# tusen-ai/simpledet

Measured on AMD Instinct MI355X. Metric: images/sec at 800x1333 FPN 512-RoI RoIAlign fwd+bwd, higher is better.
Workload: dtype f32; 1 GPU; fused FPN RoIAlign_v2 fwd+bwd, P2-P5 256ch 800x1333, N=2 img/GPU, 512 RoIs/img, 7x7x4 samples (BASELINE configs[1]); images_per_gpu=2, rois_per_image=512, argmax_state=packed u8 (decoded in backward)

## Files before the change

simpledet_amd/csrc/roi_align_common.h:

```cpp
#pragma once
#include "common.h"
#include "../../include/simpledet_ops.h"
#include <float.h>
#include <math.h>
#include <type_traits>
#include <hip/hip_fp16.h>

namespace sd {

struct RoiLevels {
  const float* data[SD_MAX_FPN_LEVELS];
  int H[SD_MAX_FPN_LEVELS], W[SD_MAX_FPN_LEVELS], stride[SD_MAX_FPN_LEVELS];
  float scale[SD_MAX_FPN_LEVELS];
  int nlvl;
  float canon_scale, canon_level, k_min, k_max;
};

__device__ __forceinline__ int fpn_level(float x1, float y1, float x2, float y2,
                                         const RoiLevels& L) {
  float area = (x2 - x1 + 1.f) * (y2 - y1 + 1.f);
  float s = sqrtf(area);
  float t = floorf(L.canon_level + log2f(s / L.canon_scale + 1e-6f));
  t = t < L.k_min ? L.k_min : (t > L.k_max ? L.k_max : t);
  if (!(t == t)) return -1;
// ... 86 lines not shown
  float* coords;
  int nslice;
  int fbslice;
  int ablate;
  long long* dbg;
  int half_io;
};

__device__ __forceinline__ int axis_samples(int p, int pooled, float start_c, float end_c,
                                            float scale, int size, int mul, float* val, float* frac,
                                            int* off) {
  float roi_start = start_c * scale;
  float roi_end = end_c * scale;
  float roi_len = roi_end - roi_start;
  float bin = roi_len / (float)pooled;
  float lo = (float)p * bin;
  float hi = (float)(p + 1) * bin;
  lo = fminr(fmaxr(lo + roi_start, 0.f), (float)(size - 1));
  hi = fminr(fmaxr(hi + roi_start, 0.f), (float)(size - 1));
  int cnt = -1;
  off[0] = off[1] = off[2] = off[3] = -1;
  if (!(hi <= lo)) {
    cnt = 0;
    float stride = (hi - lo) / 3.0f;
    double lim = (double)(hi - stride) + 0.01;
    float step = fmaxr(stride, 0.01f);
    for (float v = lo + stride; (double)v <= lim; v += step) {
      if (cnt < 2) {
        int low = iminr(imaxr((int)floorf(v), 0), size - 1);
        int high = iminr(imaxr((int)ceilf(v), 0), size - 1);
        val[cnt] = v;
        frac[cnt] = (low == high) ? 0.5f : (v - (float)low);
        off[2 * cnt] = low * mul;
        off[2 * cnt + 1] = high * mul;
      }
      ++cnt;
      if (cnt >= 3) break;
    }
  }
  return cnt;
}

constexpr int kCoordWords = 9;

__device__ __forceinline__ float sample_coord(int p, int pooled, float start_c, float end_c,
                                              float scale, int size, int k) {
  const float roi_start = start_c * scale;
  const float roi_end = end_c * scale;
  const float roi_len = roi_end - roi_start;
  const float bin = roi_len / (float)pooled;
  float lo = (float)p * bin;
  float hi = (float)(p + 1) * bin;
  lo = fminr(fmaxr(lo + roi_start, 0.f), (float)(size - 1));
  hi = fminr(fmaxr(hi + roi_start, 0.f), (float)(size - 1));
  const float stride = (hi - lo) / 3.0f;
  const float step = fmaxr(stride, 0.01f);
  float v = lo + stride;
  for (int i = 0; i < k; ++i) v += step;
  return v;
}

__device__ __forceinline__ void store_tap(float* dst, float v, int size) {
  int packed = -1;
  float frac = 0.f;
  if (v != -1.f) {
    const int lo = iminr(imaxr((int)floorf(v), 0), size - 1);
    const int hi = iminr(imaxr((int)ceilf(v), 0), size - 1);
    frac = (lo == hi) ? 0.5f : (v - (float)lo) / (float)(hi - lo);
    packed = lo | (hi << 16);
  }
  reinterpret_cast<int*>(dst)[0] = packed;
  dst[1] = frac;
}

constexpr int kBandThreads = 1024, kBandWaves = kBandThreads / kWave;
constexpr int kBandBufFloats = 16896;
constexpr int kBandHalo = 8;
constexpr int kBandMaxBands = 16;
constexpr int kBandNP = 4;
constexpr int kBandMaxUnits = 512;
constexpr int kBandFillCost = 140, kBandPlaneCost = 60, kBandSetupCost = 1500;
constexpr int kBandSub = 4;
constexpr int kBandFallbackWGs = 0;

typedef float v2f __attribute__((ext_vector_type(2)));

struct BandPlan {
  int owned[SD_MAX_FPN_LEVELS];
  int rows[SD_MAX_FPN_LEVELS];
  int nbands[SD_MAX_FPN_LEVELS];
  int g[SD_MAX_FPN_LEVELS];
  int unit_base[SD_MAX_FPN_LEVELS];
  int halo[SD_MAX_FPN_LEVELS];
  int nwg;
  int nunits;
  int grab;
  int gbias;
  int tail;
  int tail_planes;
  int pool;
  uint4* rowent;
  uint4* colent;
  float2* rowval;
  float2* colval;
  unsigned* items;
  int2* seg;
  unsigned char* fbflag;
  int* chan_ctr;
  int nlist, nent;
};

struct BandArgs {
  FwdArgs f;
  BandPlan p;
};

struct BwdArgs {
  RoiLevels L;
  const float* dy;
  const float* ax;
  const float* ay;
  const float* rois;
  float* dx;
  int B, C, R, PP, H, W;
  float scale;
  int filter_lvl;
  int band_rows, nbands;
  int req;
  int ablate;
};

struct BwdFusedArgs {
  RoiLevels L;
  const float* dy;
  const float* ax;
  const float* ay;
  const unsigned char* amax8;
  const float* coords;
  const float* rois;
  float* dx[SD_MAX_FPN_LEVELS];
  int band_rows[SD_MAX_FPN_LEVELS], nbands[SD_MAX_FPN_LEVELS];
  int block_end[SD_MAX_FPN_LEVELS];
  int order[SD_MAX_FPN_LEVELS];
  int nlaunch;
  int B, C, R, PP;
  int filter;
  int req;
  int ablate;
  int* ws_list;
  float* ws_taps;
  int unit_base[SD_MAX_FPN_LEVELS];
  int lists_units;
  int half_io;
  int float_adds;
  int pix_bound_words;
};
constexpr int kPixBoundMaxWords = 10240;

constexpr int kListSplit = 4;
constexpr int kMergedListSplit = 2;

int fill_levels(RoiLevels& L, const float* const* feats, const int* Hs, const int* Ws, const int* strides,
                int nlvl, float canon_scale, float canon_level);
int check_dims(int B, int C, int R, int ph, int pw);
int launch_fwd(FwdArgs& a, hipStream_t st, void* workspace = nullptr, size_t workspace_bytes = 0,
               const BwdFusedArgs* bplan = nullptr, bool* bplan_done = nullptr);
int launch_bwd_fused(BwdFusedArgs& a, int nlvl, hipStream_t st, void* workspace = nullptr,
                     size_t workspace_bytes = 0, int prepass = 0);
int launch_bwd(BwdArgs& a, hipStream_t st);
int launch_fwd_prep(const BandArgs& A, int pool, int nblocks, const BwdFusedArgs* bplan, hipStream_t st);
int launch_bwd_lists(const BwdFusedArgs& a, int units, hipStream_t st);

}
```

simpledet_amd/csrc/roi_align_fwd.hip:

```cpp
#include "roi_align_common.h"

namespace sd {

__global__ __launch_bounds__(256) void roi_align_fwd_naive(FwdArgs a) {
  const int PP = a.PH * a.PW;
  const long count = (long)a.B * a.R * a.C * PP;
  for (long index = (long)blockIdx.x * blockDim.x + threadIdx.x; index < count;
       index += (long)gridDim.x * blockDim.x) {
    int pw = (int)(index % a.PW);
    int ph = (int)((index / a.PW) % a.PH);
    int c = (int)((index / PP) % a.C);
    int n = (int)(index / PP / a.C);
    const float* r = a.rois + (long)n * 4;
    float x1 = r[0], y1 = r[1], x2 = r[2], y2 = r[3];
    int lvl = 0;
    if (a.L.nlvl > 1) lvl = fpn_level(x1, y1, x2, y2, a.L);
    FwdOut o{0.f, -1.f, -1.f, 255};
    if (lvl >= 0) {
      int H = a.L.H[lvl], W = a.L.W[lvl];
      const float* plane = a.L.data[lvl] + ((long)(n / a.R) * a.C + c) * H * W;
      o = roi_align_fwd_elem(plane, H, W, x1, y1, x2, y2, a.L.scale[lvl], ph, pw, a.PH, a.PW);
    }
    if (a.L.nlvl > 1) o.val = o.val + 0.0f;
    a.out[index] = o.val;
// ... 349 lines not shown
                      bk = (kl >> 1) * 3 + (kl & 1);
                    } else {
                      bx = cx[b][kl & 1];
                      by = cy[b][kl >> 1];
                    }
                  }
                }
                if (a.L.nlvl > 1) maxval = maxval + 0.0f;
                const int g = bin;
                po[g + d * NWAVE * PPG] = maxval;
                if (PK) {
                  if (!(SD_ABLATE(a, 4))) pk[g + d * NWAVE * PPSG] = (unsigned char)(bk < 0 ? 255 : bk);
                } else {
                  px[g + d * NWAVE * PPG] = bx;
                  py[g + d * NWAVE * PPG] = by;
                }
              }
            }
            wave_lds_sync();
          }
        }
        pl += D * pstep;
        po += D * NWAVE * PPG;
        if (PK) {
          pk += D * NWAVE * PPSG;
        } else {
          px += D * NWAVE * PPG;
          py += D * NWAVE * PPG;
        }
      }
    };
    if (any_dup) channel_loop(std::true_type{});
    else channel_loop(std::false_type{});
  }
}

template <int PH, int PW, int NROI, bool PK>
__global__ __launch_bounds__(512) void roi_align_fwd_tiled(FwdArgs a) {
  __shared__ FwdSmem<PH, PW, NROI> s;
  fwd_tiled_body<PH, PW, NROI, PK>(a, s, blockIdx.x);
}

__device__ __forceinline__ int band_fill(const float* gsrc, int len, float* buf, int wave, int lane) {
  const int shift = (int)(((uintptr_t)gsrc >> 2) & 3);
  const float* a0 = gsrc - shift;
  const int n4 = (shift + len + 3) >> 2;
  const int first_full = shift ? 1 : 0;
  const int last_full = ((shift + len) >> 2);
  const float4* s4 = reinterpret_cast<const float4*>(a0);
  float4* d4 = reinterpret_cast<float4*>(buf);
  for (int w4 = wave * kWave; w4 < last_full; w4 += kBandWaves * kWave) {
    const int i = w4 + lane;
    if (i >= first_full && i < last_full) __builtin_amdgcn_global_load_lds(s4 + i, d4 + w4, 16, 0, 0);
  }
  if (wave == 0) {
    if (shift && lane < 4 && lane >= shift && lane < shift + len)
      __builtin_amdgcn_global_load_lds(a0 + lane, buf, 4, 0, 0);
    if (last_full < n4 && last_full >= first_full && (last_full > 0 || !shift)) {
      const int j = last_full * 4 + lane;
      if (lane < 4 && j < shift + len) __builtin_amdgcn_global_load_lds(a0 + j, buf + last_full * 4, 4, 0, 0);
    }
  }
  return shift;
}

template <int POOL, bool PK, bool HALF = false>
__global__ __launch_bounds__(kBandThreads) void roi_align_fwd_band(BandArgs A) {
  using TIn = typename std::conditional<HALF, __half, float>::type;
  constexpr int AL = HALF ? 8 : 4;
  const FwdArgs& a = A.f;
  const BandPlan& P = A.p;
  constexpr int QL = POOL, IPP = kWave / QL;
  constexpr int NP = (PK && !HALF) ? kBandNP : kBandNP - 1, CAP = NP * kBandWaves * IPP;
  constexpr int PPG = POOL * POOL, PPSG = amax_stride(PPG);
  extern __shared__ __attribute__((aligned(16))) float band_smem[];
  const int tid = threadIdx.x, lane = tid & (kWave - 1);
  const int wave = __builtin_amdgcn_readfirstlane(tid / kWave);

#ifdef SD_PROFILING
  const long long t_entry = __builtin_readcyclecounter();
#endif
  __shared__ int v_unit[kBandMaxUnits], v_first[kBandMaxUnits], v_items[kBandMaxUnits];
  __shared__ int v_cost[kBandMaxUnits], v_start[kBandMaxUnits + 1];
  __shared__ int2 s_grab[2];
  __shared__ int s_pick;
  const int wg = (int)blockIdx.x - kBandFallbackWGs, nwg = (int)gridDim.x - kBandFallbackWGs;
  const int rsub = (a.R + kBandSub - 1) / kBandSub;
  auto level_of = [&](int u) {
    int l = 0;
    for (int k = 0; k < a.L.nlvl; ++k)
      if (a.L.stride[k] >= 0 && u >= P.unit_base[k]) l = k;
    return l;
  };
  __shared__ int s_nvu;
  auto wave_incl_scan = [&](int v) {
#pragma unroll
    for (int o = 1; o < kWave; o <<= 1) {
      const int t = __shfl_up(v, o);
      if (lane >= o) v += t;
    }
    return v;
  };
  static_assert(kBandMaxUnits % kWave == 0 && kBandMaxUnits / kWave <= kBandWaves, "unit table: one wave per 64 units");
  constexpr int NB = kBandMaxUnits / kWave;
  __shared__ int s_tot[NB], s_ctot[NB];
  {
    const int u = wave * kWave + lane;
    int cnt = 0, rounds = 0, lv = 0, incl = 0;
    if (wave < NB) {
      if (u < P.nunits) {
        lv = level_of(u);
#pragma unroll
        for (int j = 0; j < kBandSub; ++j) cnt += P.seg[u * kBandSub + j].y;
        rounds = (cnt + CAP - 1) / CAP;
      }
      incl = wave_incl_scan(rounds);
      if (lane == kWave - 1) s_tot[wave] = incl;
    }
    __syncthreads();
    int total = 0;
#pragma unroll
    for (int b = 0; b < NB; ++b) total += s_tot[b];
    const int n = total < kBandMaxUnits ? total : kBandMaxUnits;
    if (wave < NB) {
      int vb = incl - rounds;
#pragma unroll
      for (int b = 0; b < NB; ++b) vb += b < wave ? s_tot[b] : 0;
      for (int r = 0; r < rounds && vb + r < kBandMaxUnits; ++r) {
        const int it = cnt - r * CAP < CAP ? cnt - r * CAP : CAP;
        v_unit[vb + r] = u;
        v_first[vb + r] = r * CAP;
        v_items[vb + r] = it;
        const int cst = kBandFillCost / P.g[lv] + kBandPlaneCost + it;
        v_cost[vb + r] = P.g[lv] > 1 ? cst + cst * P.gbias / 100 : cst;
      }
    }
    __syncthreads();
    const int v = wave * kWave + lane;
    int mine = 0, cincl = 0;
    if (wave < NB) {
      mine = v < n ? kBandSetupCost + v_cost[v] * a.C : 0;
      cincl = wave_incl_scan(mine);
      if (lane == kWave - 1) s_ctot[wave] = cincl;
    }
    __syncthreads();
    if (wave < NB) {
      int run = cincl - mine;
#pragma unroll
      for (int b = 0; b < NB; ++b) run += b < wave ? s_ctot[b] : 0;
      if (v < n) v_start[v] = run;
      if (v == n - 1 || (n == 0 && v == 0)) v_start[n] = n == 0 ? 0 : run + mine;
    }
    if (tid == 0) s_nvu = n;
  }
  __syncthreads();
  const int nvu = s_nvu;
  int vu = 0;
  {
    const long pos = (long)v_start[nvu] * (2 * wg + 1) / (2 * nwg);
    int below = 0;
    for (int k = lane; k < nvu; k += kWave) below += v_start[k] <= pos ? 1 : 0;
    below = wave_sum_i32(below);
    vu = below > 0 ? below - 1 : 0;
  }
  float* buf0 = band_smem;
  float* buf1 = band_smem + kBandBufFloats;
#ifdef SD_PROFILING
  const long long t_begin = __builtin_readcyclecounter();
  long long t_setup = 0, t_wait = 0, t_comp = 0, t_mark = t_begin;
  int dbg_count = 0, dbg_units = 0, dbg_fills = 0;
#endif
  auto grab = [&](int v, int G) {
    int k = 0;
    if (tid == 0) k = atomicAdd(&P.chan_ctr[v], G);
    return k;
  };

  for (int visit = 0; nvu > 0; ++visit) {
  if (visit) {
    if (wave == 0) {
      int best = -1, bestval = 0;
      for (int v0 = 0; v0 < nvu; v0 += kWave) {
        const int v = v0 + lane;
        int left = 0;
        if (v < nvu) {
          const int done = __hip_atomic_load(&P.chan_ctr[v], __ATOMIC_RELAXED, __HIP_MEMORY_SCOPE_AGENT);
          if (done < a.C && (done == 0 || a.C - done >= 3 * P.g[level_of(v_unit[v])])) {
            left = (a.C - done) * v_cost[v];
            left = left < 1 ? 1 : left;
          }
        }
        int m = left;
#pragma unroll
        for (int o = 32; o >= 1; o >>= 1) {
          const int t = __shfl_xor(m, o);
          m = t > m ? t : m;
        }
        if (m > bestval) {
          bestval = m;
          best = v0 + __builtin_ctzll(__ballot(left == m));
        }
      }
      if (lane == 0) s_pick = best;
    }
    __syncthreads();
    vu = s_pick;
    if (vu < 0) break;
  }
  const int unit = v_unit[vu];
  const int lvl = level_of(unit);
  const int G = P.g[lvl], nb = P.nbands[lvl];
  const int GR = ((P.grab + G - 1) / G) * G;
  int glast = 0;
  auto next_size = [&]() { return glast >= a.C - a.C * P.tail / 100 ? (P.tail_planes < G ? P.tail_planes : G) : GR; };
  {
    const int k = grab(vu, GR);
    if (tid == 0) s_grab[0] = make_int2(k, GR);
    glast = k;
    __syncthreads();
  }
  int kcur = s_grab[0].x;
  if (kcur >= a.C) continue;
  int ck = kcur + G, cend = kcur + GR < a.C ? kcur + GR : a.C;
  int gcur = cend - kcur < G ? cend - kcur : G, gnext = 0;
  int slot = 1;
  const int ul = unit - P.unit_base[lvl];
  const int img = ul / nb, band = ul % nb;
  const int H = a.L.H[lvl], W = a.L.W[lvl], HW = H * W;
  const int r0 = band * P.owned[lvl];
  const int nrows = H - r0 < P.rows[lvl] ? H - r0 : P.rows[lvl];
  const int blen = nrows * W;
  const int bstride = HALF ? ((blen + 14) >> 3) * 8 : (blen + 4 + 3) & ~3;
  const unsigned* items = P.items + ((long)img * SD_MAX_FPN_LEVELS + lvl) * kBandSub * rsub * POOL;
  int sgs[kBandSub], sgc[kBandSub], count = 0;
#pragma unroll
  for (int j = 0; j < kBandSub; ++j) {
    const int2 sg = P.seg[unit * kBandSub + j];
    sgs[j] = j * rsub * POOL + sg.x - count;
    sgc[j] = count + sg.y;
    count += sg.y;
  }
  const int round0 = v_first[vu], nitems = v_items[vu];
#ifdef SD_PROFILING
  dbg_count += nitems;
  ++dbg_units;
  dbg_fills = 0;
  t_mark = __builtin_readcyclecounter();
  if (a.dbg && lane == 0 && wave == 0 && dbg_units <= 3) {
    long long* d = a.dbg + ((long)gridDim.x * kBandWaves + (long)blockIdx.x * 4 + (dbg_units - 1)) * 8;
    d[0] = lvl; d[2] = nitems; d[3] = t_mark; d[4] = 1;
  }
#endif
  const TIn* gbase = reinterpret_cast<const TIn*>(a.L.data[lvl]) + (long)img * a.C * HW + (long)r0 * W;
  {
    constexpr int NST = HALF ? 3 : 1;
    uint4 st[NST];
    const int n8u = (blen + 7 + 7) >> 3;
    auto fill = [&](const TIn* src, float* dst, int gcount) {
      if constexpr (!HALF) {
        int sh0 = 0;
        for (int g = 0; g < gcount; ++g) {
          const int sh = band_fill(src + (long)g * HW, blen, dst + g * bstride, wave, lane);
          if (g == 0) sh0 = sh;
        }
        return sh0;
      } else {
        const int sh0 = (int)(((uintptr_t)src >> 1) & 7);
#pragma unroll
        for (int k = 0; k < NST; ++k) {
          const int f = tid + k * kBandThreads, g = f / n8u, i = f - g * n8u;
          st[k] = make_uint4(0, 0, 0, 0);
          if (g < gcount) {
            const __half* sp = src + (long)g * HW;
            const int sh = (int)(((uintptr_t)sp >> 1) & 7);
            const int e0 = 8 * i - sh;
            if (e0 >= 0 && e0 + 8 <= blen) {
              st[k] = *reinterpret_cast<const uint4*>(sp + e0);
            } else if (e0 + 8 > 0 && e0 < blen) {
              unsigned short h[8];
#pragma unroll
              for (int j = 0; j < 8; ++j)
                h[j] = (e0 + j >= 0 && e0 + j < blen) ? reinterpret_cast<const unsigned short*>(sp)[e0 + j] : 0;
              st[k] = make_uint4(h[0] | (unsigned)h[1] << 16, h[2] | (unsigned)h[3] << 16,
                                 h[4] | (unsigned)h[5] << 16, h[6] | (unsigned)h[7] << 16);
            }
          }
        }
        return sh0;
      }
    };
    auto fill_commit = [&](float* dst, int gcount) {
      if constexpr (HALF) {
#pragma unroll
        for (int k = 0; k < NST; ++k) {
          const int f = tid + k * kBandThreads, g = f / n8u, i = f - g * n8u;
          if (g < gcount) {
            const __half2* hp = reinterpret_cast<const __half2*>(&st[k]);
            const float2 p0 = __half22float2(hp[0]), p1 = __half22float2(hp[1]);
            const float2 p2 = __half22float2(hp[2]), p3 = __half22float2(hp[3]);
            float4* d = reinterpret_cast<float4*>(dst + g * bstride + 8 * i);
            d[0] = make_float4(p0.x, p0.y, p1.x, p1.y);
            d[1] = make_float4(p2.x, p2.y, p3.x, p3.y);
          }
        }
      }
    };
    int A0[NP], A1[NP], A2[NP], A3[NP], A4[NP], A5[NP], A6[NP], A7[NP];
    float al0[NP], al1[NP], be0[NP], be1[NP], cx0[NP], cx1[NP], cy0[NP], cy1[NP];
    int ooff[NP];
    unsigned aoff[NP];
    int flags[NP];
    bool anyd[NP];
    unsigned words[NP];
    uint4 res[NP], ces[NP];
#pragma unroll
    for (int i = 0; i < NP; ++i) {
      const int it = (wave + kBandWaves * i) * IPP + lane / QL;
      const bool valid = lane < IPP * QL && it < nitems;
      words[i] = 0;
      if (valid) {
// ... 414 lines not shown
  L.nlvl = nlvl;
  L.canon_scale = canon_scale;
  L.canon_level = canon_level;
  L.k_min = (float)log2((double)smin);
  L.k_max = (float)log2((double)smax);
  return SD_OK;
}

int launch_fwd(FwdArgs& a, hipStream_t st, void* workspace, size_t workspace_bytes, const BwdFusedArgs* bplan,
               bool* bplan_done) {
  if (bplan_done) *bplan_done = false;
  const long count = (long)a.B * a.R * a.C * a.PH * a.PW;
  if (count == 0) return SD_OK;
  const int variant = tuning("roi_align_fwd", 1);
  a.ablate = SD_PROF_TUNING("roi_align_fwd_ablate", 0);
  a.dbg = reinterpret_cast<long long*>(((uintptr_t)(unsigned)SD_PROF_TUNING("roi_align_dbg_hi", 0) << 32) |
                                       (uintptr_t)(unsigned)SD_PROF_TUNING("roi_align_dbg_lo", 0));
  const int nroi = a.B * a.R;
  a.nslice = 1;
  for (int d = 1; d <= a.C && d <= 8; ++d)
    if (a.C % d == 0) a.nslice = d;
  const int wantfb = a.L.nlvl > 1 ? 32 : 8;
  a.fbslice = 1;
  for (int d = 1; d <= a.C && d <= wantfb; ++d)
    if (a.C % d == 0) a.fbslice = d;
  bool wide = true;
  for (int l = 0; l < a.L.nlvl; ++l)
    if (a.L.stride[l] >= 0 && a.L.W[l] < 2) wide = false;
  if (variant == 1 && wide && ((a.PH == 7 && a.PW == 7) || (a.PH == 14 && a.PW == 14)) &&
      a.R <= 65535 && workspace && tuning("roi_align_fwd_band", 1)) {
    BandArgs A{};
    BandPlan& P = A.p;
    const int POOL = a.PH;
    bool ok = true;
    int units = 0;
    constexpr int gmax = 8;
    int nvalid_lv = 0;
    for (int l = 0; l < a.L.nlvl; ++l) nvalid_lv += a.L.stride[l] >= 0;
    for (int l = 0; l < a.L.nlvl; ++l) {
      if (a.L.stride[l] < 0) continue;
      const int H = a.L.H[l], W = a.L.W[l];
      const long HW = (long)H * W;
      if (W > 4095 || HW >= (1 << 20)) { ok = false; break; }
      int halo = kBandHalo;
      if (H <= 128) {
        halo = (H + POOL - 1) / POOL + 2;
        halo = halo < kBandHalo ? kBandHalo : (halo > 12 ? 12 : halo);
      }
      const int rb = (kBandBufFloats - 16) / W;
      if (rb < halo + 4) { ok = false; break; }
      int nbn = H <= rb ? 1 : (H + (rb - halo) - 1) / (rb - halo);
      const int cap = kBandNP * kBandWaves * (kWave / POOL);
      const long est = (long)a.R * POOL / (nvalid_lv > 0 ? nvalid_lv : 1);
      const int by_items = (int)((est * 5 + 4L * cap - 1) / (4L * cap));
      if (by_items > nbn && a.amax8) nbn = by_items;
      if (nbn > H) nbn = H;
      if (nbn > kBandMaxBands) nbn = kBandMaxBands;
      int owned = (H + nbn - 1) / nbn;
      if (nbn > 1)
        for (int o = owned; o < owned + 4 && o + halo <= rb; ++o)
          if (((long)o * W) % 4 == 0) { owned = o; break; }
      if (owned + halo > rb) owned = rb - halo;
      nbn = (H + owned - 1) / owned;
      if (nbn > kBandMaxBands) { ok = false; break; }
      P.nbands[l] = nbn;
      P.halo[l] = halo;
      P.owned[l] = nbn == 1 ? H : owned;
      P.rows[l] = nbn == 1 ? H : (owned + halo < H ? owned + halo : H);
      const long bstride = a.half_io ? (((long)P.rows[l] * W + 14) >> 3) * 8 : (((long)P.rows[l] * W + 4 + 3) & ~3L);
      int g = 1;
      for (int c = 2; c <= 8 && c <= gmax; c *= 2)
        if (a.C % c == 0 && c * bstride <= kBandBufFloats) g = c;
      if (bstride > kBandBufFloats) { ok = false; break; }
      P.g[l] = g;
      P.unit_base[l] = units;
      units += a.B * P.nbands[l];
    }
    auto al16 = [](size_t x) { return (x + 15) & ~(size_t)15; };
    const size_t ent = al16((size_t)nroi * POOL * sizeof(uint4));
    const size_t valb = a.amax8 ? 0 : al16((size_t)nroi * POOL * sizeof(float2));
    const size_t itemb = al16((size_t)a.B * SD_MAX_FPN_LEVELS * kBandSub * ((a.R + kBandSub - 1) / kBandSub) *
                              POOL * sizeof(unsigned));
    const size_t segb = al16((size_t)units * kBandSub * sizeof(int2));
    const size_t need = 16 + 2 * ent + 2 * valb + itemb + segb + al16(nroi) + kBandMaxUnits * sizeof(int);
    int wg = 0;
    P.nunits = units;
    P.grab = 4;
    P.gbias = 0;
    P.tail = 0;
    P.tail_planes = 8;
    {
      const int np = (a.amax8 && !a.half_io) ? kBandNP : kBandNP - 1;
      const long cap_launch = (long)np * kBandWaves * (kWave / POOL);
      if (units + (long)nroi * POOL / cap_launch > kBandMaxUnits) ok = false;
    }
    wg = kNumCU;
    if (ok && need <= workspace_bytes) {
      char* w = reinterpret_cast<char*>(((uintptr_t)workspace + 15) & ~(uintptr_t)15);
      P.rowent = reinterpret_cast<uint4*>(w); w += ent;
      P.colent = reinterpret_cast<uint4*>(w); w += ent;
      if (valb) {
        P.rowval = reinterpret_cast<float2*>(w); w += valb;
        P.colval = reinterpret_cast<float2*>(w); w += valb;
      }
      P.items = reinterpret_cast<unsigned*>(w); w += itemb;
      P.seg = reinterpret_cast<int2*>(w); w += segb;
      P.fbflag = reinterpret_cast<unsigned char*>(w); w += al16(nroi);
      P.chan_ctr = reinterpret_cast<int*>(w);
      P.nwg = wg;
      P.pool = POOL;
      A.f = a;
      const int nlist = a.B * a.L.nlvl * kBandSub, nent = cdiv((long)nroi * 2 * POOL, kBandThreads);
      const int ncoord = a.amax8 ? cdiv((long)nroi * 6 * POOL, kBandThreads) : 0;
      P.nlist = nlist; P.nent = nent;
      const int smem = 2 * kBandBufFloats * (int)sizeof(float);
      const bool merged = bplan && bplan->lists_units > 0 && bplan->PP == POOL * POOL;
      if (bplan_done) *bplan_done = merged;
      if (int e = launch_fwd_prep(A, POOL, nlist + nent + ncoord, merged ? bplan : nullptr, st)) return e;
      {
        const long HW0 = (long)a.L.H[0] * a.L.W[0];
        const size_t lds = (size_t)(HW0 + 1) * 16 + 8 * 4 * 49 * sizeof(float);
        if (!a.amax8 && !a.half_io && POOL == 7 && a.L.nlvl == 1 && a.L.stride[0] >= 0 && P.nbands[0] == 1 &&
            a.C % 4 == 0 && lds <= 78 * 1024 && a.B <= 65535 &&
            (((uintptr_t)a.L.data[0] | (uintptr_t)a.out | (uintptr_t)a.ax | (uintptr_t)a.ay) & 15) == 0 &&
            tuning("roi_align_fwd_quad", 1) == 1) {
          SD_HIP_CHECK(hipFuncSetAttribute((const void*)roi_align_fwd_quad, hipFuncAttributeMaxDynamicSharedMemorySize, (int)lds));
          hipLaunchKernelGGL(roi_align_fwd_quad, dim3(a.C / 4, a.B), dim3(512), lds, st, A);
          note_dispatch("sd::roi_fwd_prep_kernel<7> + sd::roi_align_fwd_quad");
          SD_LAUNCH_CHECK();
          return SD_OK;
        }
      }
#define SD_FWD_BAND(POOLV, PK)                                                                    \
  do {                                                                                            \
    auto k = roi_align_fwd_band<POOLV, PK>;                                                       \
    SD_HIP_CHECK(hipFuncSetAttribute((const void*)k, hipFuncAttributeMaxDynamicSharedMemorySize,  \
                                     smem));                                                      \
    hipLaunchKernelGGL(k, dim3(wg + kBandFallbackWGs), dim3(kBandThreads), smem, st, A);          \
  } while (0)
      if (a.half_io) {
#define SD_FWD_BAND_H(POOLV)                                                                      \
  do {                                                                                            \
    auto k = roi_align_fwd_band<POOLV, true, true>;                                               \
    SD_HIP_CHECK(hipFuncSetAttribute((const void*)k, hipFuncAttributeMaxDynamicSharedMemorySize,  \
                                     smem));                                                      \
    hipLaunchKernelGGL(k, dim3(wg + kBandFallbackWGs), dim3(kBandThreads), smem, st, A);          \
  } while (0)
        if (POOL == 7) SD_FWD_BAND_H(7); else SD_FWD_BAND_H(14);
#undef SD_FWD_BAND_H
      } else if (POOL == 7) {
        if (a.amax8) SD_FWD_BAND(7, true); else SD_FWD_BAND(7, false);
      } else {
        if (a.amax8) SD_FWD_BAND(14, true); else SD_FWD_BAND(14, false);
      }
#undef SD_FWD_BAND
      note_dispatch("sd::%s<%d> + sd::roi_align_fwd_band<%d,%s,%s>", merged ? "roi_prep_merged_kernel" : "roi_fwd_prep_kernel",
                    POOL, POOL, a.amax8 ? "true" : "false", a.half_io ? "true" : "false");
      SD_LAUNCH_CHECK();
      return SD_OK;
    }
  }
  if (a.half_io)
    return fail(SD_ERR_UNSUPPORTED, "fp16 RoIAlign runs on the band-resident kernel only: it needs the workspace, "
                "7x7 or 14x14 pooling, W in [2, 4095] and roi_align_fwd = 1, roi_align_fwd_band = 1");
  note_dispatch("sd::roi_align_fwd (tiled / naive fallback kernels: no workspace or a shape the band kernel does not take)");
  if (variant >= 1 && wide && a.PH == 7 && a.PW == 7) {
    if (a.amax8)
      hipLaunchKernelGGL((roi_align_fwd_tiled<7, 7, 4, true>), dim3(cdiv(nroi, 4) * a.nslice), dim3(512), 0, st, a);
    else
      hipLaunchKernelGGL((roi_align_fwd_tiled<7, 7, 4, false>), dim3(cdiv(nroi, 4) * a.nslice), dim3(512), 0, st, a);
  } else if (variant >= 1 && wide && a.PH == 14 && a.PW == 14) {
    if (a.amax8)
      hipLaunchKernelGGL((roi_align_fwd_tiled<14, 14, 1, true>), dim3(nroi * a.nslice), dim3(512), 0,
                         st, a);
    else
      hipLaunchKernelGGL((roi_align_fwd_tiled<14, 14, 1, false>), dim3(nroi * a.nslice), dim3(512),
                         0, st, a);
  } else {
    const int grid = (int)((count + 255) / 256 < 65536 * 16 ? (count + 255) / 256 : 65536 * 16);
    hipLaunchKernelGGL(roi_align_fwd_naive, dim3(grid), dim3(256), 0, st, a);
    if (a.amax8)
      hipLaunchKernelGGL(roi_coords_kernel, dim3(nroi), dim3(64), 0, st, a.rois, nroi, a.L, a.PH,
                         a.PW, a.coords);
  }
  SD_LAUNCH_CHECK();
  return SD_OK;
}

int check_dims(int B, int C, int R, int ph, int pw) {
  SD_REQUIRE(B >= 0 && C >= 0 && R >= 0, "negative dimension (B=%d C=%d R=%d)", B, C, R);
  SD_REQUIRE(ph > 0 && pw > 0, "pooled_size must be nonzero (got %d x %d)", ph, pw);
// ... 77 lines not shown
  FwdArgs a{};
  if (int e = fill_levels(a.L, feats_host, Hs_host, Ws_host, strides_host, nlvl,
                          roi_canonical_scale, roi_canonical_level))
    return e;
  for (int l = 0; l < nlvl; ++l) SD_REQUIRE(feats_host[l] || (long)B * C == 0, "feats[%d] null", l);
  if (nlvl == 1) a.L.nlvl = 2, a.L.stride[1] = -1;
  a.rois = rois; a.out = out; a.amax8 = argmax; a.coords = coords;
  a.B = B; a.C = C; a.R = R; a.PH = pooled_h; a.PW = pooled_w;
  hipStream_t st = (hipStream_t)stream;
  BwdFusedArgs f{};
  bool have = false;
  if (plan && ((uintptr_t)plan & 15) == 0 && (long)B * R * C > 0 && R <= 8192 &&
      ((pooled_h == 7 && pooled_w == 7) || (pooled_h == 14 && pooled_w == 14))) {
    f.L = a.L;
    f.amax8 = argmax; f.coords = coords; f.rois = rois;
    for (int l = 0; l < nlvl; ++l) f.dx[l] = reinterpret_cast<float*>(uintptr_t(16));
    f.B = B; f.C = C; f.R = R; f.PP = pooled_h * pooled_w; f.filter = 1; f.req = SD_REQ_WRITE;
    have = launch_bwd_fused(f, nlvl, st, plan, plan_bytes, 1) == SD_OK;
  }
  bool done = false;
  if (int e = launch_fwd(a, st, workspace, workspace_bytes, have ? &f : nullptr, &done)) return e;
  if (have && !done)
    if (int e = launch_bwd_lists(f, f.lists_units, st)) return e;
  return SD_OK;
}

extern "C" int sd_fpn_roi_align_fwd_packed(const float* const* feats_host, const int* Hs_host,
                                           const int* Ws_host, const int* strides_host, int nlvl,
                                           const float* rois, float* out, uint8_t* argmax,
                                           float* coords, int B, int C, int R, int pooled_h,
                                           int pooled_w,
                                           float roi_canonical_scale, float roi_canonical_level,
                                           void* workspace, size_t workspace_bytes, void* stream) {
  return fpn_fwd_packed_impl(feats_host, Hs_host, Ws_host, strides_host, nlvl, rois, out, argmax, coords, B, C,
                             R, pooled_h, pooled_w, roi_canonical_scale, roi_canonical_level, workspace,
                             workspace_bytes, nullptr, 0, stream);
}

extern "C" int sd_fpn_roi_align_fwd_packed_plan(const float* const* feats_host, const int* Hs_host,
                                                const int* Ws_host, const int* strides_host, int nlvl,
                                                const float* rois, float* out, uint8_t* argmax,
                                                float* coords, int B, int C, int R, int pooled_h,
                                                int pooled_w, float roi_canonical_scale,
                                                float roi_canonical_level, void* workspace,
                                                size_t workspace_bytes, void* plan, size_t plan_bytes,
                                                void* stream) {
  SD_REQUIRE(plan, "plan is null (use sd_fpn_roi_align_fwd_packed)");
  SD_REQUIRE(((uintptr_t)plan & 15) == 0, "plan must be 16-byte aligned");
  return fpn_fwd_packed_impl(feats_host, Hs_host, Ws_host, strides_host, nlvl, rois, out, argmax, coords, B, C,
                             R, pooled_h, pooled_w, roi_canonical_scale, roi_canonical_level, workspace,
                             workspace_bytes, plan, plan_bytes, stream);
}

extern "C" int sd_fpn_roi_align_fwd_packed_f16(const void* const* feats_host, const int* Hs_host,
                                               const int* Ws_host, const int* strides_host, int nlvl,
                                               const float* rois, void* out, uint8_t* argmax,
                                               float* coords, int B, int C, int R, int pooled_h,
                                               int pooled_w, float roi_canonical_scale,
                                               float roi_canonical_level, void* workspace,
                                               size_t workspace_bytes, void* stream) {
  if (int e = check_dims(B, C, R, pooled_h, pooled_w)) return e;
  SD_REQUIRE(feats_host && Hs_host && Ws_host && strides_host, "null level description");
  SD_REQUIRE((argmax && coords && out) || (long)B * R * C == 0, "out / argmax / coords is null");
  SD_REQUIRE(((uintptr_t)argmax & 3) == 0 && ((uintptr_t)coords & 7) == 0 && ((uintptr_t)out & 1) == 0,
             "argmax must be 4-byte, coords 8-byte and out 2-byte aligned");
  FwdArgs a{};
  if (int e = fill_levels(a.L, reinterpret_cast<const float* const*>(feats_host), Hs_host, Ws_host,
                          strides_host, nlvl, roi_canonical_scale, roi_canonical_level))
    return e;
  for (int l = 0; l < nlvl; ++l) {
    SD_REQUIRE(feats_host[l] || (long)B * C == 0, "feats[%d] null", l);
    SD_REQUIRE(((uintptr_t)feats_host[l] & 15) == 0, "feats[%d] must be 16-byte aligned", l);
  }
  if (nlvl == 1) a.L.nlvl = 2, a.L.stride[1] = -1;
  a.rois = rois; a.out = reinterpret_cast<float*>(out); a.amax8 = argmax; a.coords = coords;
  a.B = B; a.C = C; a.R = R; a.PH = pooled_h; a.PW = pooled_w;
  a.half_io = 1;
  return launch_fwd(a, (hipStream_t)stream, workspace, workspace_bytes);
}

extern "C" size_t sd_fpn_roi_align_workspace_bytes(int B, int R) {
  const size_t b = B > 0 ? B : 0, r = R > 0 ? R : 0, nroi = b * r;
  return nroi * 14 * (2 * 16 + 2 * 8) + b * SD_MAX_FPN_LEVELS * (r + kBandSub) * 14 * 4 +
         b * SD_MAX_FPN_LEVELS * kBandMaxBands * kBandSub * 8 + nroi + kBandMaxUnits * 4 + 256;
}

extern "C" int sd_fpn_roi_assign(const float* rois, int n_rois, const int* strides_host, int nlvl,
                                 float roi_canonical_scale, float roi_canonical_level,
                                 float* rois_per_level, int32_t* level, void* stream) {
  SD_REQUIRE(n_rois >= 0, "n_rois < 0");
  SD_REQUIRE(strides_host, "strides null");
  RoiLevels L{};
  int ones[SD_MAX_FPN_LEVELS];
  for (int l = 0; l < SD_MAX_FPN_LEVELS; ++l) ones[l] = 1;
  if (int e = fill_levels(L, nullptr, ones, ones, strides_host, nlvl, roi_canonical_scale,
                          roi_canonical_level))
    return e;
  if (n_rois == 0) return SD_OK;
  SD_REQUIRE(rois, "rois null");
  hipLaunchKernelGGL(fpn_assign_kernel, dim3(cdiv(n_rois, 256)), dim3(256), 0,
                     (hipStream_t)stream, rois, n_rois, L, rois_per_level, level);
  SD_LAUNCH_CHECK();
  return SD_OK;
}
```

simpledet_amd/csrc/roi_align_prep.hip:

```cpp
#include "roi_align_lists.h"

namespace sd {

template <int POOL>
__device__ __forceinline__ void band_prep_block(const BandArgs& A, const int pblock, int nlist, int nent) {
  const FwdArgs& a = A.f;
  const BandPlan& P = A.p;
  const int tid = threadIdx.x, lane = tid & (kWave - 1);
  constexpr int LPR = POOL <= 8 ? 8 : 16;
  constexpr int RPP = kBandThreads / LPR;
  if (pblock < nlist) {
    __shared__ int hist[kBandMaxBands], cursor[kBandMaxBands];
    const int sub = pblock % kBandSub, lvl = (pblock / kBandSub) % a.L.nlvl;
    const int img = pblock / (kBandSub * a.L.nlvl);
    if (a.L.stride[lvl] < 0) return;
    int first_valid = 0;
    while (a.L.stride[first_valid] < 0) ++first_valid;
    const int H = a.L.H[lvl], W = a.L.W[lvl], nb = P.nbands[lvl], owned = P.owned[lvl];
    const float scale = a.L.scale[lvl];
    const int rsub = (a.R + kBandSub - 1) / kBandSub;
    const int rbeg = sub * rsub, rend = rbeg + rsub < a.R ? rbeg + rsub : a.R;
    if (tid < kBandMaxBands) hist[tid] = 0;
    __syncthreads();
    const int rr = tid / LPR, p = tid % LPR;
    unsigned* items = P.items + (((long)img * SD_MAX_FPN_LEVELS + lvl) * kBandSub + sub) * rsub * POOL;
    auto classify = [&](int n) -> int {
      int band = -1;
      bool bad = false, mine = false, emp_r = true, emp_c = true;
      int lv = -2;
      if (n < rend) {
        const float4 bx = *reinterpret_cast<const float4*>(a.rois + ((long)img * a.R + n) * 4);
        lv = a.L.nlvl > 1 ? fpn_level(bx.x, bx.y, bx.z, bx.w, a.L) : 0;
        mine = lv == lvl;
        if (mine && p < POOL) {
          float val[2], frac[2];
          int offr[4], offc[4];
          const int cr = axis_samples(p, POOL, bx.y, bx.w, scale, H, 1, val, frac, offr);
          const int cc = axis_samples(p, POOL, bx.x, bx.z, scale, W, 1, val, frac, offc);
          bad = cr >= 3 || cc >= 3;
          emp_r = cr < 0;
          emp_c = cc < 0;
          band = 0;
          if (cr >= 1) {
            const int first = offr[0], last = cr >= 2 ? offr[3] : offr[1];
            if (nb > 1 && last - first > P.halo[lvl]) bad = true;
            band = first / owned;
          }
        }
      }
      const unsigned long long bm = __ballot(bad);
      const int sh = (lane / LPR) * LPR;
      const unsigned long long rmask = (1ull << LPR) - 1;
      bool roi_bad = ((bm >> sh) & rmask) != 0;
      const bool all_r = ((__ballot(!emp_r) >> sh) & rmask) == 0, all_c = ((__ballot(!emp_c) >> sh) & rmask) == 0;
      const bool roi_void = mine && (all_r || all_c);
      roi_bad = roi_bad || roi_void;
      if (n < rend && p == 0) {
        if (mine) P.fbflag[(long)img * a.R + n] = roi_void ? 2 : (roi_bad ? 1 : 0);
        else if (lv < 0 && lvl == first_valid) P.fbflag[(long)img * a.R + n] = 2;
      }
      return roi_bad ? -2 : band;
    };
    constexpr int KP = 4;
    int keep[KP];
    const int npass = (rend - rbeg + RPP - 1) / RPP;
#pragma unroll
    for (int k = 0; k < KP; ++k) {
      keep[k] = -1;
      if (k < npass) {
        keep[k] = classify(rbeg + k * RPP + rr);
        if (keep[k] >= 0) atomicAdd(&hist[keep[k]], 1);
      }
    }
    for (int k = KP; k < npass; ++k) {
      const int band = classify(rbeg + k * RPP + rr);
      if (band >= 0) atomicAdd(&hist[band], 1);
    }
    __syncthreads();
    if (tid == 0) {
      int run = 0;
      for (int b = 0; b < nb; ++b) {
        cursor[b] = run;
        P.seg[(P.unit_base[lvl] + img * nb + b) * kBandSub + sub] = make_int2(run, hist[b]);
        run += hist[b];
      }
    }
    __syncthreads();
    auto emit = [&](int n, int band) {
      unsigned long long todo = __ballot(band >= 0);
      while (todo) {
        const int src = __builtin_ctzll(todo);
        const int bb = __builtin_amdgcn_readlane(band, src);
        const unsigned long long m = __ballot(band == bb);
        int base = 0;
        if (lane == src) base = atomicAdd(&cursor[bb], __popcll(m));
        base = __builtin_amdgcn_readlane(base, src);
        if (band == bb)
          items[base + __builtin_amdgcn_mbcnt_hi((unsigned)(m >> 32), __builtin_amdgcn_mbcnt_lo((unsigned)m, 0))] =
              (unsigned)n | ((unsigned)p << 16);
        todo &= ~m;
      }
    };
#pragma unroll
    for (int k = 0; k < KP; ++k)
      if (k < npass) emit(rbeg + k * RPP + rr, keep[k]);
    for (int k = KP; k < npass; ++k) {
      const int n = rbeg + k * RPP + rr;
      emit(n, classify(n));
    }
    return;
  }
  if (pblock == nlist && tid < kBandMaxUnits) P.chan_ctr[tid] = 0;
  const int eb = pblock - nlist;
  const int nroi = a.B * a.R;
  if (eb < nent) {
    const long e = (long)eb * kBandThreads + tid;
    if (e >= (long)nroi * 2 * POOL) return;
    const int p = (int)(e % POOL), ax = (int)((e / POOL) % 2), n = (int)(e / (2 * POOL));
    const float4 bx = *reinterpret_cast<const float4*>(a.rois + (long)n * 4);
    const int lvl = a.L.nlvl > 1 ? fpn_level(bx.x, bx.y, bx.z, bx.w, a.L) : 0;
    if (lvl < 0) return;
    const int H = a.L.H[lvl], W = a.L.W[lvl];
    float val[2] = {0.f, 0.f}, frac[2] = {0.f, 0.f};
    int off[4];
    const int cnt = ax == 0 ? axis_samples(p, POOL, bx.y, bx.w, a.L.scale[lvl], H, W, val, frac, off)
                            : axis_samples(p, POOL, bx.x, bx.z, a.L.scale[lvl], W, 1, val, frac, off);
    const float qnan = __int_as_float(0x7fc00000);
    const bool v0 = cnt >= 1, v1 = cnt >= 2;
    uint4 en;
    if (ax == 0) {
      en.x = (v0 ? (unsigned)off[0] | (off[1] != off[0] ? 1u << 20 : 0u) : 0u) | (cnt < 0 ? 1u << 31 : 0u);
      en.y = v1 ? (unsigned)off[2] | (off[3] != off[2] ? 1u << 20 : 0u) : 0u;
    } else {
      en.x = (v0 ? (unsigned)off[0] | (off[1] == off[0] ? 1u << 12 : 0u) : 0u) |
             (v1 ? (unsigned)off[2] << 13 | (off[3] == off[2] ? 1u << 25 : 0u) : 0u) | (cnt < 0 ? 1u << 26 : 0u);
      en.y = 0u;
    }
    en.z = __float_as_uint(v0 ? frac[0] : qnan);
    en.w = __float_as_uint(v1 ? frac[1] : qnan);
    (ax == 0 ? P.rowent : P.colent)[(long)n * POOL + p] = en;
    if (P.rowval) (ax == 0 ? P.rowval : P.colval)[(long)n * POOL + p] = make_float2(val[0], val[1]);
    return;
  }
  if (a.amax8) {
    const long e = (long)(eb - nent) * kBandThreads + tid;
    if (e >= (long)nroi * 6 * POOL) return;
    const int j = (int)(e % (6 * POOL)), n = (int)(e / (6 * POOL));
    const float4 bx = *reinterpret_cast<const float4*>(a.rois + (long)n * 4);
    const int lvl = a.L.nlvl > 1 ? fpn_level(bx.x, bx.y, bx.z, bx.w, a.L) : 0;
    if (lvl < 0) return;
    const bool row = j < 3 * POOL;
    const int jj = row ? j : j - 3 * POOL;
    const float v = row ? sample_coord(jj / 3, POOL, bx.y, bx.w, a.L.scale[lvl], a.L.H[lvl], jj % 3)
                        : sample_coord(jj / 3, POOL, bx.x, bx.z, a.L.scale[lvl], a.L.W[lvl], jj % 3);
    float* cb = a.coords + (long)n * kCoordWords * (POOL + POOL);
    cb[j] = v;
    store_tap(cb + 3 * (POOL + POOL) + 2 * j, v, row ? a.L.H[lvl] : a.L.W[lvl]);
  }
}

template <int POOL>
__global__ __launch_bounds__(kBandThreads) void roi_fwd_prep_kernel(BandArgs A) {
  band_prep_block<POOL>(A, (int)blockIdx.x, A.p.nlist, A.p.nent);
}

template <int PH, int PW, int THREADS, int PARTS>
__device__ __forceinline__ void bwd_lists_block(const BwdFusedArgs& a, int block, float* smem) {
  int* list = reinterpret_cast<int*>(smem);
  int* nlist = list + a.R;
  const int tid = threadIdx.x;
  const int NP = PARTS + (a.pix_bound_words > 0 ? 1 : 0);
  const int unit = block / NP, part = block % NP;
  int li = 0;
  while (li + 1 < a.nlaunch && unit >= a.unit_base[li + 1]) ++li;
  const int lvl = a.order[li];
  const int u = unit - a.unit_base[li];
  const int nbands = a.nbands[lvl];
  const int img = u / nbands, band = u % nbands;
  const int row0 = band * a.band_rows[lvl];
  const int row1 = iminr(row0 + a.band_rows[lvl], a.L.H[lvl]);
  float4 rb0 = make_float4(0.f, 0.f, 0.f, 0.f);
  if (tid < a.R) rb0 = *reinterpret_cast<const float4*>(a.rois + ((long)img * a.R + tid) * 4);
  if (tid < 8) nlist[tid] = 0;
  __syncthreads();
  bwd_band_list<PH, PW, THREADS>(a, lvl, img, nbands, row0, row1, rb0, list, nlist, nlist + 8);
  int* dst = a.ws_list + (long)unit * (a.R + 2);
  const int nl = nlist[0];
  const int H = a.L.H[lvl], W = a.L.W[lvl];
  constexpr int CS = 2;
  const int DW = ((W - 1) >> CS) + 2, DH = ((row1 - row0 - 1) >> CS) + 2;
  const bool pix = DW * DH <= a.pix_bound_words;
  if (part == 0) {
// ... 126 lines not shown
```

Before: 10330 images/s.

## Build band schedule once in prep kernel instead of per workgroup

Result: no change. 10260 images/s (-0.7%).

```diff
diff --git a/simpledet_amd/csrc/roi_align_common.h b/simpledet_amd/csrc/roi_align_common.h
--- a/simpledet_amd/csrc/roi_align_common.h
+++ b/simpledet_amd/csrc/roi_align_common.h
@@ -192,6 +192,9 @@
 constexpr int kBandFillCost = 140, kBandPlaneCost = 60, kBandSetupCost = 1500;
 constexpr int kBandSub = 4;
 constexpr int kBandFallbackWGs = 0;
+__host__ __device__ constexpr int band_cap(int pool, bool packed, bool half_io) {
+  return ((packed && !half_io) ? kBandNP : kBandNP - 1) * kBandWaves * (kWave / pool);
+}
 
 typedef float v2f __attribute__((ext_vector_type(2)));
 
@@ -218,7 +221,18 @@
   unsigned char* fbflag;
   int* chan_ctr;
   int nlist, nent;
-};
+  int cap;
+  int4* vrow;
+  int* vstart;
+  unsigned long long* sched_ctl;
+};
+
+__device__ __forceinline__ int band_level_of(const BandPlan& P, const RoiLevels& L, int u) {
+  int l = 0;
+  for (int k = 0; k < L.nlvl; ++k)
+    if (L.stride[k] >= 0 && u >= P.unit_base[k]) l = k;
+  return l;
+}
 
 struct BandArgs {
   FwdArgs f;
diff --git a/simpledet_amd/csrc/roi_align_fwd.hip b/simpledet_amd/csrc/roi_align_fwd.hip
--- a/simpledet_amd/csrc/roi_align_fwd.hip
+++ b/simpledet_amd/csrc/roi_align_fwd.hip
@@ -455,79 +455,38 @@
 #endif
   __shared__ int v_unit[kBandMaxUnits], v_first[kBandMaxUnits], v_items[kBandMaxUnits];
   __shared__ int v_cost[kBandMaxUnits], v_start[kBandMaxUnits + 1];
+  __shared__ int2 s_seg[kBandMaxUnits * kBandSub];
   __shared__ int2 s_grab[2];
   __shared__ int s_pick;
   const int wg = (int)blockIdx.x - kBandFallbackWGs, nwg = (int)gridDim.x - kBandFallbackWGs;
   const int rsub = (a.R + kBandSub - 1) / kBandSub;
-  auto level_of = [&](int u) {
-    int l = 0;
-    for (int k = 0; k < a.L.nlvl; ++k)
-      if (a.L.stride[k] >= 0 && u >= P.unit_base[k]) l = k;
-    return l;
-  };
-  __shared__ int s_nvu;
-  auto wave_incl_scan = [&](int v) {
-#pragma unroll
-    for (int o = 1; o < kWave; o <<= 1) {
-      const int t = __shfl_up(v, o);
-      if (lane >= o) v += t;
-    }
-    return v;
-  };
-  static_assert(kBandMaxUnits % kWave == 0 && kBandMaxUnits / kWave <= kBandWaves, "unit table: one wave per 64 units");
-  constexpr int NB = kBandMaxUnits / kWave;
-  __shared__ int s_tot[NB], s_ctot[NB];
+  auto level_of = [&](int u) { return band_level_of(P, a.L, u); };
+  static_assert(kBandThreads == 2 * kBandMaxUnits && kBandMaxUnits * kBandSub == 2 * kBandThreads, "table load: one trip");
+  static_assert(CAP == band_cap(POOL, PK, HALF), "the pre-pass cuts rounds of band_cap items");
+  int nvu;
   {
-    const int u = wave * kWave + lane;
-    int cnt = 0, rounds = 0, lv = 0, incl = 0;
-    if (wave < NB) {
-      if (u < P.nunits) {
-        lv = level_of(u);
-#pragma unroll
-        for (int j = 0; j < kBandSub; ++j) cnt += P.seg[u * kBandSub + j].y;
-        rounds = (cnt + CAP - 1) / CAP;
-      }
-      incl = wave_incl_scan(rounds);
-      if (lane == kWave - 1) s_tot[wave] = incl;
-    }
-    __syncthreads();
-    int total = 0;
-#pragma unroll
-    for (int b = 0; b < NB; ++b) total += s_tot[b];
-    const int n = total < kBandMaxUnits ? total : kBandMaxUnits;
-    if (wave < NB) {
-      int vb = incl - rounds;
-#pragma unroll
-      for (int b = 0; b < NB; ++b) vb += b < wave ? s_tot[b] : 0;
-      for (int r = 0; r < rounds && vb + r < kBandMaxUnits; ++r) {
-        const int it = cnt - r * CAP < CAP ? cnt - r * CAP : CAP;
-        v_unit[vb + r] = u;
-        v_first[vb + r] = r * CAP;
-        v_items[vb + r] = it;
-        const int cst = kBandFillCost / P.g[lv] + kBandPlaneCost + it;
-        v_cost[vb + r] = P.g[lv] > 1 ? cst + cst * P.gbias / 100 : cst;
-      }
-    }
-    __syncthreads();
-    const int v = wave * kWave + lane;
-    int mine = 0, cincl = 0;
-    if (wave < NB) {
-      mine = v < n ? kBandSetupCost + v_cost[v] * a.C : 0;
-      cincl = wave_incl_scan(mine);
-      if (lane == kWave - 1) s_ctot[wave] = cincl;
-    }
-    __syncthreads();
-    if (wave < NB) {
-      int run = cincl - mine;
-#pragma unroll
-      for (int b = 0; b < NB; ++b) run += b < wave ? s_ctot[b] : 0;
-      if (v < n) v_start[v] = run;
-      if (v == n - 1 || (n == 0 && v == 0)) v_start[n] = n == 0 ? 0 : run + mine;
-    }
-    if (tid == 0) s_nvu = n;
+    nvu = P.vstart[kBandMaxUnits + 1];
+    int4 row = make_int4(0, 0, 0, 0);
+    int st = 0, st_end = 0;
+    if (tid < kBandMaxUnits) row = P.vrow[tid];
+    else st = P.vstart[tid - kBandMaxUnits];
+    if (tid == kBandThreads - 1) st_end = P.vstart[kBandMaxUnits];
+    const int nseg = P.nunits * kBandSub;
+    int2 sg0 = make_int2(0, 0), sg1 = sg0;
+    if (tid < nseg) sg0 = P.seg[tid];
+    if (tid + kBandThreads < nseg) sg1 = P.seg[tid + kBandThreads];
+    if (tid < kBandMaxUnits) {
+      v_unit[tid] = row.x; v_first[tid] = row.y; v_items[tid] = row.z; v_cost[tid] = row.w;
+    } else {
+      v_start[tid - kBandMaxUnits] = st;
+    }
+    if (tid == kBandThreads - 1) v_start[kBandMaxUnits] = st_end;
+    s_seg[tid] = sg0;
+    s_seg[tid + kBandThreads] = sg1;
+    nvu = __builtin_amdgcn_readfirstlane(nvu);
+    nvu = nvu < 0 ? 0 : (nvu > kBandMaxUnits ? kBandMaxUnits : nvu);
   }
   __syncthreads();
-  const int nvu = s_nvu;
   int vu = 0;
   {
     const long pos = (long)v_start[nvu] * (2 * wg + 1) / (2 * nwg);
@@ -552,16 +511,23 @@
   for (int visit = 0; nvu > 0; ++visit) {
   if (visit) {
     if (wave == 0) {
+      constexpr int NB = kBandMaxUnits / kWave;
+      int done[NB];
+#pragma unroll
+      for (int b = 0; b < NB; ++b) {
+        const int v = b * kWave + lane;
+        done[b] = a.C;
+        if (v < nvu) done[b] = __hip_atomic_load(&P.chan_ctr[v], __ATOMIC_RELAXED, __HIP_MEMORY_SCOPE_AGENT);
+      }
       int best = -1, bestval = 0;
-      for (int v0 = 0; v0 < nvu; v0 += kWave) {
-        const int v = v0 + lane;
+#pragma unroll
+      for (int b = 0; b < NB; ++b) {
+        if (b * kWave >= nvu) break;
+        const int v = b * kWave + lane;
         int left = 0;
-        if (v < nvu) {
-          const int done = __hip_atomic_load(&P.chan_ctr[v], __ATOMIC_RELAXED, __HIP_MEMORY_SCOPE_AGENT);
-          if (done < a.C && (done == 0 || a.C - done >= 3 * P.g[level_of(v_unit[v])])) {
-            left = (a.C - done) * v_cost[v];
-            left = left < 1 ? 1 : left;
-          }
+        if (v < nvu && done[b] < a.C && (done[b] == 0 || a.C - done[b] >= 3 * P.g[level_of(v_unit[v])])) {
+          left = (a.C - done[b]) * v_cost[v];
+          left = left < 1 ? 1 : left;
         }
         int m = left;
 #pragma unroll
@@ -571,7 +537,7 @@
         }
         if (m > bestval) {
           bestval = m;
-          best = v0 + __builtin_ctzll(__ballot(left == m));
+          best = b * kWave + __builtin_ctzll(__ballot(left == m));
         }
       }
       if (lane == 0) s_pick = best;
@@ -608,7 +574,7 @@
   int sgs[kBandSub], sgc[kBandSub], count = 0;
 #pragma unroll
   for (int j = 0; j < kBandSub; ++j) {
-    const int2 sg = P.seg[unit * kBandSub + j];
+    const int2 sg = s_seg[unit * kBandSub + j];
     sgs[j] = j * rsub * POOL + sg.x - count;
     sgc[j] = count + sg.y;
     count += sg.y;
@@ -1189,7 +1155,9 @@
     const size_t itemb = al16((size_t)a.B * SD_MAX_FPN_LEVELS * kBandSub * ((a.R + kBandSub - 1) / kBandSub) *
                               POOL * sizeof(unsigned));
     const size_t segb = al16((size_t)units * kBandSub * sizeof(int2));
-    const size_t need = 16 + 2 * ent + 2 * valb + itemb + segb + al16(nroi) + kBandMaxUnits * sizeof(int);
+    const size_t vrowb = kBandMaxUnits * sizeof(int4), vstartb = al16((kBandMaxUnits + 2) * sizeof(int));
+    const size_t need = 16 + 2 * ent + 2 * valb + itemb + segb + al16(nroi) + kBandMaxUnits * sizeof(int) + vrowb +
+                        vstartb + 16;
     int wg = 0;
     P.nunits = units;
     P.grab = 4;
@@ -1197,9 +1165,9 @@
     P.tail = 0;
     P.tail_planes = 8;
     {
-      const int np = (a.amax8 && !a.half_io) ? kBandNP : kBandNP - 1;
-      const long cap_launch = (long)np * kBandWaves * (kWave / POOL);
-      if (units + (long)nroi * POOL / cap_launch > kBandMaxUnits) ok = false;
+      P.cap = band_cap(POOL, a.amax8 != nullptr, a.half_io != 0);
+      if (units + (long)nroi * POOL / P.cap > kBandMaxUnits) ok = false;
+      if ((long)a.B * a.L.nlvl * kBandSub > 0xffff) ok = false;
     }
     wg = kNumCU;
     if (ok && need <= workspace_bytes) {
@@ -1213,7 +1181,10 @@
       P.items = reinterpret_cast<unsigned*>(w); w += itemb;
       P.seg = reinterpret_cast<int2*>(w); w += segb;
       P.fbflag = reinterpret_cast<unsigned char*>(w); w += al16(nroi);
-      P.chan_ctr = reinterpret_cast<int*>(w);
+      P.chan_ctr = reinterpret_cast<int*>(w); w += kBandMaxUnits * sizeof(int);
+      P.vrow = reinterpret_cast<int4*>(w); w += vrowb;
+      P.vstart = reinterpret_cast<int*>(w); w += vstartb;
+      P.sched_ctl = reinterpret_cast<unsigned long long*>(w);
       P.nwg = wg;
       P.pool = POOL;
       A.f = a;
@@ -1457,7 +1428,8 @@
 extern "C" size_t sd_fpn_roi_align_workspace_bytes(int B, int R) {
   const size_t b = B > 0 ? B : 0, r = R > 0 ? R : 0, nroi = b * r;
   return nroi * 14 * (2 * 16 + 2 * 8) + b * SD_MAX_FPN_LEVELS * (r + kBandSub) * 14 * 4 +
-         b * SD_MAX_FPN_LEVELS * kBandMaxBands * kBandSub * 8 + nroi + kBandMaxUnits * 4 + 256;
+         b * SD_MAX_FPN_LEVELS * kBandMaxBands * kBandSub * 8 + nroi + kBandMaxUnits * 4 +
+         kBandMaxUnits * 16 + (kBandMaxUnits + 2) * 4 + 16 + 256;
 }
 
 extern "C" int sd_fpn_roi_assign(const float* rois, int n_rois, const int* strides_host, int nlvl,
diff --git a/simpledet_amd/csrc/roi_align_prep.hip b/simpledet_amd/csrc/roi_align_prep.hip
--- a/simpledet_amd/csrc/roi_align_prep.hip
+++ b/simpledet_amd/csrc/roi_align_prep.hip
@@ -1,6 +1,85 @@
 #include "roi_align_lists.h"
 
 namespace sd {
+
+__device__ __forceinline__ void band_seg_store(int2* seg, int first, int count) {
+  __hip_atomic_store(reinterpret_cast<unsigned long long*>(seg),
+                     (unsigned long long)(unsigned)first | (unsigned long long)(unsigned)count << 32, __ATOMIC_RELAXED,
+                     __HIP_MEMORY_SCOPE_AGENT);
+}
+__device__ __forceinline__ bool band_sched_tick(unsigned long long* ctl, int nlist) {
+  const unsigned long long ep = __hip_atomic_load(&ctl[0], __ATOMIC_RELAXED, __HIP_MEMORY_SCOPE_AGENT);
+  const unsigned long long tag = (ep * 0x9E3779B97F4A7C15ull + 0x7F4A7C15ull) & ~0xffffull;
+  const unsigned long long cur = __hip_atomic_load(&ctl[1], __ATOMIC_RELAXED, __HIP_MEMORY_SCOPE_AGENT);
+  asm volatile("s_waitcnt vmcnt(0)" ::: "memory");
+  if ((cur & ~0xffffull) != tag) {
+    unsigned long long expect = cur;
+    __hip_atomic_compare_exchange_strong(&ctl[1], &expect, tag, __ATOMIC_RELAXED, __ATOMIC_RELAXED, __HIP_MEMORY_SCOPE_AGENT);
+  }
+  const unsigned long long nxt = __hip_atomic_fetch_add(&ctl[1], 1ull, __ATOMIC_RELAXED, __HIP_MEMORY_SCOPE_AGENT) + 1;
+  return (int)(nxt & 0xffff) == nlist;
+}
+
+__device__ __forceinline__ void band_build_schedule(const BandArgs& A) {
+  const FwdArgs& a = A.f;
+  const BandPlan& P = A.p;
+  static_assert(kBandMaxUnits % kWave == 0 && kBandMaxUnits / kWave <= kBandWaves, "unit table: one wave per 64 units");
+  constexpr int NB = kBandMaxUnits / kWave;
+  __shared__ int s_tot[NB], s_ctot[NB], s_cost[kBandMaxUnits];
+  const int tid = threadIdx.x, lane = tid & (kWave - 1), wave = tid / kWave;
+  const int CAP = P.cap;
+  const int u = wave * kWave + lane;
+  int cnt = 0, rounds = 0, lv = 0, incl = 0;
+  if (wave < NB) {
+    if (u < P.nunits) {
+      lv = band_level_of(P, a.L, u);
+#pragma unroll
+      for (int j = 0; j < kBandSub; ++j)
+        cnt += (int)(__hip_atomic_load(reinterpret_cast<unsigned long long*>(&P.seg[u * kBandSub + j]), __ATOMIC_RELAXED,
+                                       __HIP_MEMORY_SCOPE_AGENT) >> 32);
+      rounds = (cnt + CAP - 1) / CAP;
+    }
+    incl = wave_scan_i32(rounds);
+    if (lane == kWave - 1) s_tot[wave] = incl;
+  }
+  __syncthreads();
+  int total = 0;
+#pragma unroll
+  for (int b = 0; b < NB; ++b) total += s_tot[b];
+  const int n = total < kBandMaxUnits ? total : kBandMaxUnits;
+  if (wave < NB) {
+    int vb = incl - rounds;
+#pragma unroll
+    for (int b = 0; b < NB; ++b) vb += b < wave ? s_tot[b] : 0;
+    for (int r = 0; r < rounds && vb + r < kBandMaxUnits; ++r) {
+      const int it = cnt - r * CAP < CAP ? cnt - r * CAP : CAP;
+      const int cst = kBandFillCost / P.g[lv] + kBandPlaneCost + it;
+      const int cost = P.g[lv] > 1 ? cst + cst * P.gbias / 100 : cst;
+      s_cost[vb + r] = cost;
+      P.vrow[vb + r] = make_int4(u, r * CAP, it, cost);
+    }
+  }
+  __syncthreads();
+  const int v = wave * kWave + lane;
+  int mine = 0, cincl = 0;
+  if (wave < NB) {
+    mine = v < n ? kBandSetupCost + s_cost[v] * a.C : 0;
+    cincl = wave_scan_i32(mine);
+    if (lane == kWave - 1) s_ctot[wave] = cincl;
+  }
+  __syncthreads();
+  if (wave < NB) {
+    int run = cincl - mine;
+#pragma unroll
+    for (int b = 0; b < NB; ++b) run += b < wave ? s_ctot[b] : 0;
+    if (v < n) P.vstart[v] = run;
+    if (v == n - 1 || (n == 0 && v == 0)) P.vstart[n] = n == 0 ? 0 : run + mine;
+  }
+  if (tid == 0) {
+    P.vstart[kBandMaxUnits + 1] = n;
+    P.sched_ctl[0] = __hip_atomic_load(&P.sched_ctl[0], __ATOMIC_RELAXED, __HIP_MEMORY_SCOPE_AGENT) + 1;
+  }
+}
 
 template <int POOL>
 __device__ __forceinline__ void band_prep_block(const BandArgs& A, const int pblock, int nlist, int nent) {
@@ -11,9 +90,15 @@
   constexpr int RPP = kBandThreads / LPR;
   if (pblock < nlist) {
     __shared__ int hist[kBandMaxBands], cursor[kBandMaxBands];
+    __shared__ int s_last;
     const int sub = pblock % kBandSub, lvl = (pblock / kBandSub) % a.L.nlvl;
     const int img = pblock / (kBandSub * a.L.nlvl);
-    if (a.L.stride[lvl] < 0) return;
+    if (a.L.stride[lvl] < 0) {
+      if (tid == 0) s_last = band_sched_tick(P.sched_ctl, nlist) ? 1 : 0;
+      __syncthreads();
+      if (s_last) band_build_schedule(A);
+      return;
+    }
     int first_valid = 0;
     while (a.L.stride[first_valid] < 0) ++first_valid;
     const int H = a.L.H[lvl], W = a.L.W[lvl], nb = P.nbands[lvl], owned = P.owned[lvl];
@@ -22,6 +107,7 @@
     const int rbeg = sub * rsub, rend = rbeg + rsub < a.R ? rbeg + rsub : a.R;
     if (tid < kBandMaxBands) hist[tid] = 0;
     __syncthreads();
+    bool last_tick = false;
     const int rr = tid / LPR, p = tid % LPR;
     unsigned* items = P.items + (((long)img * SD_MAX_FPN_LEVELS + lvl) * kBandSub + sub) * rsub * POOL;
     auto classify = [&](int n) -> int {
@@ -81,9 +167,10 @@
       int run = 0;
       for (int b = 0; b < nb; ++b) {
         cursor[b] = run;
-        P.seg[(P.unit_base[lvl] + img * nb + b) * kBandSub + sub] = make_int2(run, hist[b]);
+        band_seg_store(&P.seg[(P.unit_base[lvl] + img * nb + b) * kBandSub + sub], run, hist[b]);
         run += hist[b];
       }
+      last_tick = band_sched_tick(P.sched_ctl, nlist);
     }
     __syncthreads();
     auto emit = [&](int n, int band) {
@@ -108,6 +195,9 @@
       const int n = rbeg + k * RPP + rr;
       emit(n, classify(n));
     }
+    if (tid == 0) s_last = last_tick ? 1 : 0;
+    __syncthreads();
+    if (s_last) band_build_schedule(A);
     return;
   }
   if (pblock == nlist && tid < kBandMaxUnits) P.chan_ctr[tid] = 0;
```
